# VainF/Diff-Pruning

Measured on NVIDIA H100. Metric: taylor_score_unet_fwd_bwd_passes_per_sec, higher is better.
Workload: dtype f32

## Files before the change

diff-pruning_b200/csrc/conv_tc.cu:

```cuda
#include <cuda.h>
#include <cuda_fp16.h>
#include <mutex>
#include "common.cuh"
#include "sm90.cuh"

namespace {
using namespace sm90;

constexpr int BM = 128, BK = 64;
constexpr int A_BYTES = BM * 32 * 4;

struct TcParams {
  int Nimg, H, W;
  int Nout;
  int kchunks;
  int bw, bh, bn, tiles_w, tiles_h;
  float* y; long long ldy;
  const float* bias;
  const float* rowadd; long long ld_rowadd;
  const float* residual; long long ld_res;
  int accumulate;
  int vec4;
  int ntaps;
  signed char dh[9], dw[9], wt[9];
  int os, oa, ob, Ho, Wo;
  int in_stride;
  float alpha;
  int b_from_img;
  const uint32_t* amax_a;
  const uint32_t* amax_b;
  uint32_t* amax_out;
  int ksplit, it_per_split;
  float* ws; long long ws_split_stride; int ws_ld;
};

__device__ __forceinline__ uint32_t smem_u32(const void* p) { return (uint32_t)__cvta_generic_to_shared(p); }
__device__ __forceinline__ void mbar_init(uint32_t bar, uint32_t count) {
  asm volatile("mbarrier.init.shared::cta.b64 [%0], %1;" ::"r"(bar), "r"(count));
}
__device__ __forceinline__ void mbar_expect_tx(uint32_t bar, uint32_t bytes) {
  asm volatile("mbarrier.arrive.expect_tx.shared::cta.b64 _, [%0], %1;" ::"r"(bar), "r"(bytes) : "memory");
}
__device__ __forceinline__ void mbar_arrive(uint32_t bar) {
  asm volatile("mbarrier.arrive.shared::cta.b64 _, [%0];" ::"r"(bar) : "memory");
}
__device__ __forceinline__ void mbar_wait(uint32_t bar, uint32_t parity) {
  uint32_t done;
  do {
    asm volatile(
        "{\n\t.reg .pred p;\n\t"
        "mbarrier.try_wait.parity.shared::cta.b64 p, [%1], %2;\n\t"
        "selp.u32 %0, 1, 0, p;\n\t}"
        : "=r"(done)
        : "r"(bar), "r"(parity)
        : "memory");
  } while (!done);
}
__device__ __forceinline__ void tma_load_4d(uint32_t dst, const CUtensorMap* map, uint32_t bar, int c0, int c1, int c2, int c3) {
  asm volatile(
      "cp.async.bulk.tensor.4d.shared::cluster.global.mbarrier::complete_tx::bytes [%0], [%1, {%3, %4, %5, %6}], [%2];"
      ::"r"(dst), "l"(reinterpret_cast<uint64_t>(map)), "r"(bar), "r"(c0), "r"(c1), "r"(c2), "r"(c3)
      : "memory");
}
__device__ __forceinline__ void tma_load_3d(uint32_t dst, const CUtensorMap* map, uint32_t bar, int c0, int c1, int c2) {
  asm volatile(
      "cp.async.bulk.tensor.3d.shared::cluster.global.mbarrier::complete_tx::bytes [%0], [%1, {%3, %4, %5}], [%2];"
      ::"r"(dst), "l"(reinterpret_cast<uint64_t>(map)), "r"(bar), "r"(c0), "r"(c1), "r"(c2)
      : "memory");
}
__device__ __forceinline__ int amax_exponent(const uint32_t* slot) {
  const int E = (int)((__ldg(slot) >> 23) & 0xFFu);
  return min(max(E, 14), 254);
}
__device__ __forceinline__ float scale_up(int E) { return __uint_as_float((uint32_t)(267 - E) << 23); }
__device__ __forceinline__ float scale_dn(int E) { return __uint_as_float((uint32_t)(E - 13) << 23); }
constexpr float LO_SCALE = 2048.f, LO_UNSCALE = 1.f / 2048.f;
__device__ __forceinline__ void split2(float a, float b, uint32_t& h, uint32_t& l) {
  const __half2 hh = __floats2half2_rn(a, b);
  const float2 hf = __half22float2(hh);
  const __half2 ll = __floats2half2_rn((a - hf.x) * LO_SCALE, (b - hf.y) * LO_SCALE);
  h = *reinterpret_cast<const uint32_t*>(&hh);
  l = *reinterpret_cast<const uint32_t*>(&ll);
}
__device__ __forceinline__ void split1(float v, __half& h, __half& l) {
  h = __float2half_rn(v);
  l = __float2half_rn((v - __half2float(h)) * LO_SCALE);
}

constexpr int PS_STAGES = 3, PS_BN = 128;
constexpr int PS_B_BYTES = PS_BN * BK * 2;
constexpr int PS_STAGE_BYTES = 2 * A_BYTES + 2 * PS_B_BYTES;

__global__ void __launch_bounds__(THREADS, 1)
conv_tc_ps_kernel(const __grid_constant__ CUtensorMap mapA, const __grid_constant__ CUtensorMap mapBh,
                  const __grid_constant__ CUtensorMap mapBl, const TcParams p, const int tiles_m, const int total_tiles) {
  const int total_work = total_tiles * p.ksplit;
  extern __shared__ uint8_t smem_raw[];
  const uint32_t raw = smem_u32(smem_raw);
  const uint32_t pad_to = ((raw + 1023u) & ~1023u) - raw;
  uint8_t* smem = smem_raw + pad_to;
  const uint32_t sbase = raw + pad_to;
  const uint32_t bar0 = sbase + PS_STAGES * PS_STAGE_BYTES;
  auto full_bar = [&](int s) { return bar0 + 8u * s; };
  auto empty_bar = [&](int s) { return bar0 + 8u * (PS_STAGES + s); };
  const int wg = threadIdx.x >> 7, tid = threadIdx.x & 127;
  if (threadIdx.x == 0) {
    for (int s = 0; s < PS_STAGES; ++s) { mbar_init(full_bar(s), 1); mbar_init(empty_bar(s), 8); }
    mbar_init_fence();
  }
  __syncthreads();
  const int iters_per_tile = p.ntaps * p.kchunks;

  auto tile_coords = [&](int tile, int& q0, int& p0, int& n0, int& nblk) {
    nblk = tile / tiles_m;
    const int tile_m = tile - nblk * tiles_m;
    const int tw = tile_m % p.tiles_w;
    const int th = (tile_m / p.tiles_w) % p.tiles_h;
    const int tn = tile_m / (p.tiles_w * p.tiles_h);
    q0 = tw * p.bw; p0 = th * p.bh; n0 = tn * p.bn;
  };

  if (wg == 0) {
    setmaxnreg_dec<40>();
    if (threadIdx.x == 0) {
      prefetch_map(&mapA); prefetch_map(&mapBh); prefetch_map(&mapBl);
      uint32_t g = 0;
      for (int wi = blockIdx.x; wi < total_work; wi += gridDim.x) {
        const int tile = wi % total_tiles, it0 = (wi / total_tiles) * p.it_per_split, it1 = min(iters_per_tile, it0 + p.it_per_split);
        int q0, p0, n0, nblk;
        tile_coords(tile, q0, p0, n0, nblk);
        for (int it = it0; it < it1; ++it, ++g) {
          const int s = g % PS_STAGES;
          const uint32_t ph = (g / PS_STAGES) & 1u;
          mbar_wait(empty_bar(s), ph ^ 1u);
          mbar_expect_tx(full_bar(s), PS_STAGE_BYTES);
          const int tap = it / p.kchunks, kc = it - tap * p.kchunks;
          const uint32_t st = sbase + s * PS_STAGE_BYTES;
          const int aw = q0 * p.in_stride + p.dw[tap], ah = p0 * p.in_stride + p.dh[tap];
          tma_load_4d(st, &mapA, full_bar(s), kc * BK, aw, ah, n0);
          tma_load_4d(st + A_BYTES, &mapA, full_bar(s), kc * BK + 32, aw, ah, n0);
          const int tapb = p.b_from_img ? n0 : p.wt[tap];
          tma_load_3d(st + 2 * A_BYTES, &mapBh, full_bar(s), kc * BK, nblk * PS_BN, tapb);
          tma_load_3d(st + 2 * A_BYTES + PS_B_BYTES, &mapBl, full_bar(s), kc * BK, nblk * PS_BN, tapb);
        }
      }
    }
    return;
  }
  setmaxnreg_inc<232>();
  const int c = wg - 1;
  const int warp = tid >> 5, lane = tid & 31;
  const int r = 64 * c + (tid & 63), h = tid >> 6;
  const uint32_t sw = (uint32_t)(r & 7);
  const float sa = scale_up(amax_exponent(p.amax_a));
  const float f1 = scale_dn(amax_exponent(p.amax_a)), f2 = scale_dn(amax_exponent(p.amax_b)) * p.alpha;
  auto fin = [&](float main, float corr) { return fmaf(corr, LO_UNSCALE, main) * f1 * f2; };
  float amax = 0.f;
  uint32_t g = 0;
  for (int wi = blockIdx.x; wi < total_work; wi += gridDim.x) {
    const int tile = wi % total_tiles, it0 = (wi / total_tiles) * p.it_per_split, it1 = min(iters_per_tile, it0 + p.it_per_split);
    float acc[64], cor[64];
    int prev_s = 0;
    for (int it = it0; it < it1; ++it, ++g) {
      const int s = g % PS_STAGES;
      const uint32_t ph = (g / PS_STAGES) & 1u;
      mbar_wait(full_bar(s), ph);
      uint8_t* a0 = smem + s * PS_STAGE_BYTES + r * 128;
      uint8_t* a1 = a0 + A_BYTES;
      const uint8_t* src = h ? a1 : a0;
      float4 v[8];
#pragma unroll
      for (int j = 0; j < 8; ++j) v[j] = *reinterpret_cast<const float4*>(src + ((j ^ sw) << 4));
      named_sync(1 + c, 128);
#pragma unroll
      for (int m = 0; m < 4; ++m) {
        const float4 x0 = v[2 * m], x1 = v[2 * m + 1];
        uint4 hq, lq;
        split2(x0.x * sa, x0.y * sa, hq.x, lq.x);
        split2(x0.z * sa, x0.w * sa, hq.y, lq.y);
        split2(x1.x * sa, x1.y * sa, hq.z, lq.z);
        split2(x1.z * sa, x1.w * sa, hq.w, lq.w);
        const uint32_t pos = (uint32_t)(((4 * h + m) ^ sw) << 4);
        *reinterpret_cast<uint4*>(a0 + pos) = hq;
        *reinterpret_cast<uint4*>(a1 + pos) = lq;
      }
      fence_proxy_async();
      named_sync(1 + c, 128);
      const uint32_t st = sbase + s * PS_STAGE_BYTES;
      wgmma_fence();
#pragma unroll
      for (int k = 0; k < BK / 16; ++k) {
        const uint64_t a_hi = desc_k(st + c * 8192 + k * 32), a_lo = desc_k(st + A_BYTES + c * 8192 + k * 32);
        const uint64_t b_hi = desc_k(st + 2 * A_BYTES + k * 32), b_lo = desc_k(st + 2 * A_BYTES + PS_B_BYTES + k * 32);
        const uint32_t first = (it > it0 || k > 0) ? 1u : 0u;
        wgmma_f16_n128<0, 0>(acc, a_hi, b_hi, first);
        wgmma_f16_n128<0, 0>(cor, a_hi, b_lo, first);
        wgmma_f16_n128<0, 0>(cor, a_lo, b_hi, 1u);
      }
      wgmma_commit();
      wgmma_wait<1>();
      if (it > it0 && lane == 0) mbar_arrive(empty_bar(prev_s));
      prev_s = s;
    }
    wgmma_wait<0>();
    fence_regs(acc); fence_regs(cor);
    if (lane == 0) mbar_arrive(empty_bar(prev_s));

    int q0, p0, n0, nblk;
    tile_coords(tile, q0, p0, n0, nblk);
#pragma unroll
    for (int i = 0; i < 2; ++i) {
      const int row = 64 * c + 16 * warp + (lane >> 2) + 8 * i;
      const int cb = 2 * (lane & 3);
      if (p.ksplit > 1) {
        float* wrow = p.ws + (long long)(wi / total_tiles) * p.ws_split_stride + ((long long)(tile - nblk * tiles_m) * BM + row) * p.ws_ld + nblk * PS_BN;
#pragma unroll
        for (int j = 0; j < 16; ++j)
          *reinterpret_cast<float2*>(wrow + 8 * j + cb) =
              make_float2(fin(acc[4 * j + 2 * i], cor[4 * j + 2 * i]), fin(acc[4 * j + 2 * i + 1], cor[4 * j + 2 * i + 1]));
        continue;
      }
      const int w_l = row % p.bw, h_l = (row / p.bw) % p.bh, n_l = row / (p.bw * p.bh);
      const int img = n0 + n_l;
      if (img >= p.Nimg) continue;
      const long long m = ((long long)img * p.Ho + ((p0 + h_l) * p.os + p.oa)) * p.Wo + ((q0 + w_l) * p.os + p.ob);
      float* yrow = p.y + m * p.ldy;
      const float* rrow = p.residual ? p.residual + m * p.ld_res : nullptr;
      const float* arow2 = p.rowadd ? p.rowadd + (long long)img * p.ld_rowadd : nullptr;
#pragma unroll
      for (int j = 0; j < 16; ++j) {
        const int col = nblk * PS_BN + 8 * j + cb;
        float o[2] = {fin(acc[4 * j + 2 * i], cor[4 * j + 2 * i]), fin(acc[4 * j + 2 * i + 1], cor[4 * j + 2 * i + 1])};
        if (p.vec4 && col + 2 <= p.Nout) {
          if (p.bias) { const float2 t = __ldg(reinterpret_cast<const float2*>(p.bias + col)); o[0] += t.x; o[1] += t.y; }
          if (arow2) { const float2 t = __ldg(reinterpret_cast<const float2*>(arow2 + col)); o[0] += t.x; o[1] += t.y; }
          if (rrow) { const float2 t = __ldg(reinterpret_cast<const float2*>(rrow + col)); o[0] += t.x; o[1] += t.y; }
          float2* dst = reinterpret_cast<float2*>(yrow + col);
          if (p.accumulate) { const float2 t = *dst; o[0] += t.x; o[1] += t.y; }
          *dst = make_float2(o[0], o[1]);
          amax = fmaxf(amax, fmaxf(fabsf(o[0]), fabsf(o[1])));
        } else {
#pragma unroll
          for (int e = 0; e < 2; ++e) {
            const int cc = col + e;
            if (cc < p.Nout) {
              float ov = o[e];
              if (p.bias) ov += __ldg(p.bias + cc);
              if (arow2) ov += __ldg(arow2 + cc);
              if (rrow) ov += __ldg(rrow + cc);
              if (p.accumulate) ov += yrow[cc];
              yrow[cc] = ov;
              amax = fmaxf(amax, fabsf(ov));
            }
          }
        }
      }
    }
  }
  if (p.amax_out && p.ksplit == 1) amax_commit(p.amax_out, amax);
}

__global__ void __launch_bounds__(256) splitk_epilogue_kernel(const TcParams p, const int tiles_m) {
  const int c4 = (p.Nout + 3) >> 2;
  const long long total = (long long)tiles_m * BM * c4;
  float amax = 0.f;
  for (long long i = blockIdx.x * 256ll + threadIdx.x; i < total; i += (long long)gridDim.x * 256) {
    const long long grow = i / c4;
    const int c = (int)(i - grow * c4) << 2;
    const int tile_m = (int)(grow / BM), row = (int)(grow - (long long)tile_m * BM);
    const int tw = tile_m % p.tiles_w, th = (tile_m / p.tiles_w) % p.tiles_h, tn = tile_m / (p.tiles_w * p.tiles_h);
    const int w_l = row % p.bw, h_l = (row / p.bw) % p.bh, n_l = row / (p.bw * p.bh);
    const int img = tn * p.bn + n_l;
    if (img >= p.Nimg) continue;
    const float* src = p.ws + grow * p.ws_ld + c;
    float4 acc = *reinterpret_cast<const float4*>(src);
    for (int ks = 1; ks < p.ksplit; ++ks) {
      const float4 t = *reinterpret_cast<const float4*>(src + ks * p.ws_split_stride);
      acc.x += t.x; acc.y += t.y; acc.z += t.z; acc.w += t.w;
    }
    float o[4] = {acc.x, acc.y, acc.z, acc.w};
    const long long m = ((long long)img * p.Ho + ((th * p.bh + h_l) * p.os + p.oa)) * p.Wo + ((tw * p.bw + w_l) * p.os + p.ob);
    float* yrow = p.y + m * p.ldy;
#pragma unroll
    for (int e = 0; e < 4; ++e) {
      const int cc = c + e;
      if (cc < p.Nout) {
        float v = o[e];
        if (p.bias) v += __ldg(p.bias + cc);
        if (p.rowadd) v += __ldg(p.rowadd + (long long)img * p.ld_rowadd + cc);
        if (p.residual) v += __ldg(p.residual + m * p.ld_res + cc);
        if (p.accumulate) v += yrow[cc];
        yrow[cc] = v;
        amax = fmaxf(amax, fabsf(v));
      }
    }
  }
  if (p.amax_out) amax_commit(p.amax_out, amax);
}

struct WgParams {
  int Nimg, H, W, C, K;
  int R, S, pad;
  int bw, bh, bn, tiles_w, tiles_h;
  int total_chunks, chunks_per_split;
  int c_tiles;
  float* ws;
  int in_stride;
  const uint32_t* amax_x; const uint32_t* amax_y;
  float* bias_ws;
};
constexpr int WG_KPIX = 64;
constexpr int WG_BLK = WG_KPIX * 128;
constexpr int WG_STAGES = 3, WG_STAGE_BYTES = 8 * WG_BLK;

__global__ void __launch_bounds__(THREADS, 1)
wgrad_tc_kernel(const __grid_constant__ CUtensorMap mapDy, const __grid_constant__ CUtensorMap mapX, const WgParams p) {
  extern __shared__ uint8_t smem_raw[];
  const uint32_t raw = smem_u32(smem_raw);
  const uint32_t pad_to = ((raw + 1023u) & ~1023u) - raw;
  uint8_t* smem = smem_raw + pad_to;
  const uint32_t sbase = raw + pad_to;
  const uint32_t bar0 = sbase + WG_STAGES * WG_STAGE_BYTES;
  auto full_bar = [&](int s) { return bar0 + 8u * s; };
  auto empty_bar = [&](int s) { return bar0 + 8u * (WG_STAGES + s); };
  float* bsh = reinterpret_cast<float*>(smem + WG_STAGES * WG_STAGE_BYTES + 8 * 2 * WG_STAGES);
  const int wg = threadIdx.x >> 7, tid = threadIdx.x & 127;
  if (threadIdx.x == 0) {
    for (int s = 0; s < WG_STAGES; ++s) { mbar_init(full_bar(s), 1); mbar_init(empty_bar(s), 8); }
    mbar_init_fence();
  }
  __syncthreads();

  const int T = p.R * p.S;
  int tile = blockIdx.x;
  const int tap = tile % T; tile /= T;
  const int ct = tile % p.c_tiles;
  const int kt = tile / p.c_tiles;
  const int r = tap / p.S, sx = tap - r * p.S;
  const int chunk0 = blockIdx.y * p.chunks_per_split;
  const int chunk1 = min(p.total_chunks, chunk0 + p.chunks_per_split);
  const int num_iters = max(0, chunk1 - chunk0);
  const int dy_boxes = min(4, (p.K - kt * 128 + 31) >> 5), x_boxes = min(4, (p.C - ct * 128 + 31) >> 5);

  if (wg == 0) {
    setmaxnreg_dec<40>();
    if (threadIdx.x == 0) {
      prefetch_map(&mapDy); prefetch_map(&mapX);
      for (int it = 0; it < num_iters; ++it) {
        const int s = it % WG_STAGES;
        const uint32_t ph = (uint32_t)(it / WG_STAGES) & 1u;
        mbar_wait(empty_bar(s), ph ^ 1u);
        mbar_expect_tx(full_bar(s), (uint32_t)((dy_boxes + x_boxes) * WG_BLK));
        const int chunk = chunk0 + it;
        const int tw = chunk % p.tiles_w;
        const int th = (chunk / p.tiles_w) % p.tiles_h;
        const int tn = chunk / (p.tiles_w * p.tiles_h);
        const int q0 = tw * p.bw, p0 = th * p.bh, n0 = tn * p.bn;
        const uint32_t st = sbase + s * WG_STAGE_BYTES;
        const int xw = q0 * p.in_stride + sx - p.pad, xh = p0 * p.in_stride + r - p.pad;
#pragma unroll
        for (int b = 0; b < 4; ++b) {
          const uint32_t slot = (uint32_t)((b & 1) * 2 + (b >> 1));
          if (b < dy_boxes) tma_load_4d(st + slot * WG_BLK, &mapDy, full_bar(s), kt * 128 + b * 32, q0, p0, n0);
          if (b < x_boxes) tma_load_4d(st + (4 + slot) * WG_BLK, &mapX, full_bar(s), ct * 128 + b * 32, xw, xh, n0);
        }
      }
    }
    return;
  }
  setmaxnreg_inc<232>();
  const int c = wg - 1;
  const int warp = tid >> 5, lane = tid & 31;
  const int Ey = amax_exponent(p.amax_y), Ex = amax_exponent(p.amax_x);
  const float sy = scale_up(Ey), sxs = scale_up(Ex);
  const int ch = tid & 63, dh = tid >> 6;
  const bool dy_valid = ((64 * c + ch) >> 5) < dy_boxes;
  const uint32_t dy_raw = (uint32_t)((ch >> 5) * 2 + c) * WG_BLK, bl = (uint32_t)(ch & 31);
  const int xp = tid & 63, xh = tid >> 6;
  const bool x_valid = 2 * c + xh < x_boxes;
  const uint32_t xsw = (uint32_t)(xp & 7);
  float bsum = 0.f;
  float acc[64], cor[64];
  int prev_s = 0;
  for (int it = 0; it < num_iters; ++it) {
    const int s = it % WG_STAGES;
    const uint32_t ph = (uint32_t)(it / WG_STAGES) & 1u;
    mbar_wait(full_bar(s), ph);
    uint8_t* stp = smem + s * WG_STAGE_BYTES;
    float dv[32];
    if (dy_valid) {
#pragma unroll
      for (int j = 0; j < 32; ++j) {
        const int pix = 32 * dh + j;
        dv[j] = *reinterpret_cast<const float*>(stp + dy_raw + pix * 128 + ((((bl >> 2) ^ (uint32_t)pix) & 7u) << 4) + (bl & 3u) * 4);
      }
    }
    uint8_t* x0 = stp + 4 * WG_BLK + c * WG_BLK + xp * 128;
    uint8_t* x1 = x0 + 2 * WG_BLK;
    float4 xv[8];
    if (x_valid) {
      const uint8_t* src = xh ? x1 : x0;
#pragma unroll
      for (int j = 0; j < 8; ++j) xv[j] = *reinterpret_cast<const float4*>(src + ((j ^ xsw) << 4));
    }
    named_sync(1 + c, 128);
    if (dy_valid) {
      __half* dh_hi = reinterpret_cast<__half*>(stp + c * WG_BLK);
      __half* dh_lo = reinterpret_cast<__half*>(stp + (2 + c) * WG_BLK);
      float ssum = 0.f;
#pragma unroll
      for (int j = 0; j < 32; j += 2) {
        ssum += dv[j] + dv[j + 1];
#pragma unroll
        for (int e = 0; e < 2; ++e) {
          const int pix = 32 * dh + j + e;
          const int off = pix * 64 + ((((ch >> 3) ^ pix) & 7) << 3) + (ch & 7);
          split1(dv[j + e] * sy, dh_hi[off], dh_lo[off]);
        }
      }
      bsum += ssum;
    }
    if (x_valid) {
#pragma unroll
      for (int m = 0; m < 4; ++m) {
        const float4 u0 = xv[2 * m], u1 = xv[2 * m + 1];
        uint4 hq, lq;
        split2(u0.x * sxs, u0.y * sxs, hq.x, lq.x);
        split2(u0.z * sxs, u0.w * sxs, hq.y, lq.y);
        split2(u1.x * sxs, u1.y * sxs, hq.z, lq.z);
        split2(u1.z * sxs, u1.w * sxs, hq.w, lq.w);
        const uint32_t pos = (uint32_t)(((4 * xh + m) ^ xsw) << 4);
        *reinterpret_cast<uint4*>(x0 + pos) = hq;
        *reinterpret_cast<uint4*>(x1 + pos) = lq;
      }
    }
    fence_proxy_async();
    named_sync(3, 256);
    const uint32_t st = sbase + s * WG_STAGE_BYTES;
    wgmma_fence();
#pragma unroll
    for (int k = 0; k < WG_KPIX / 16; ++k) {
      const uint64_t a_hi = desc_mn(st + c * WG_BLK + k * 2048, WG_BLK), a_lo = desc_mn(st + (2 + c) * WG_BLK + k * 2048, WG_BLK);
      const uint64_t b_hi = desc_mn(st + 4 * WG_BLK + k * 2048, WG_BLK), b_lo = desc_mn(st + 6 * WG_BLK + k * 2048, WG_BLK);
      const uint32_t first = (it > 0 || k > 0) ? 1u : 0u;
      wgmma_f16_n128<1, 1>(acc, a_hi, b_hi, first);
      wgmma_f16_n128<1, 1>(cor, a_hi, b_lo, first);
      wgmma_f16_n128<1, 1>(cor, a_lo, b_hi, 1u);
    }
    wgmma_commit();
    wgmma_wait<1>();
    if (it > 0 && lane == 0) mbar_arrive(empty_bar(prev_s));
    prev_s = s;
  }
  wgmma_wait<0>();
  fence_regs(acc); fence_regs(cor);
  if (dh) bsh[64 * c + ch] = bsum;
  named_sync(3, 256);
  if (!dh) {
    bsum += bsh[64 * c + ch];
    const int kout = kt * 128 + 64 * c + ch;
    if (p.bias_ws && tap == 0 && ct == 0 && kout < p.K) p.bias_ws[(long long)blockIdx.y * p.K + kout] = bsum;
  }
  const float f1 = scale_dn(Ey), f2 = scale_dn(Ex);
  const long long TC_ = (long long)T * p.C;
#pragma unroll
  for (int i = 0; i < 2; ++i) {
    const int kout = kt * 128 + 64 * c + 16 * warp + (lane >> 2) + 8 * i;
    if (kout >= p.K) continue;
    float* wrow = p.ws + ((long long)blockIdx.y * p.K + kout) * TC_ + (long long)tap * p.C;
#pragma unroll
    for (int j = 0; j < 16; ++j)
#pragma unroll
      for (int e = 0; e < 2; ++e) {
        const int col = ct * 128 + 8 * j + 2 * (lane & 3) + e;
        if (col < p.C) wrow[col] = num_iters ? fmaf(cor[4 * j + 2 * i + e], LO_UNSCALE, acc[4 * j + 2 * i + e]) * f1 * f2 : 0.f;
      }
  }
}

typedef CUresult (*EncodeTiledFn)(CUtensorMap*, CUtensorMapDataType, cuuint32_t, void*, const cuuint64_t*, const cuuint64_t*,
                                  const cuuint32_t*, const cuuint32_t*, CUtensorMapInterleave, CUtensorMapSwizzle,
                                  CUtensorMapL2promotion, CUtensorMapFloatOOBfill);
EncodeTiledFn g_encode = nullptr;
int g_tc_state = -1;
int g_num_sms = 132;
std::mutex g_tc_mutex;
constexpr int PS_SMEM = PS_STAGES * PS_STAGE_BYTES + 2048;
constexpr int WG_SMEM = WG_STAGES * WG_STAGE_BYTES + 2048;

static int wrow(int c) { return c > 64 ? ((c + 63) & ~63) : ((c + 7) & ~7); }

int tc_init() {
  std::lock_guard<std::mutex> lk(g_tc_mutex);
  if (g_tc_state >= 0) return g_tc_state;
  g_tc_state = 0;
  int dev = 0, major = 0;
  if (cudaGetDevice(&dev) != cudaSuccess) { (void)cudaGetLastError(); return 0; }
  if (cudaDeviceGetAttribute(&major, cudaDevAttrComputeCapabilityMajor, dev) != cudaSuccess || major != 9) { (void)cudaGetLastError(); return 0; }
  void* fn = nullptr;
  cudaDriverEntryPointQueryResult qres;
  if (cudaGetDriverEntryPoint("cuTensorMapEncodeTiled", &fn, cudaEnableDefault, &qres) != cudaSuccess || !fn ||
      qres != cudaDriverEntryPointSuccess) { (void)cudaGetLastError(); return 0; }
  g_encode = (EncodeTiledFn)fn;
  bool ok = cudaFuncSetAttribute(conv_tc_ps_kernel, cudaFuncAttributeMaxDynamicSharedMemorySize, PS_SMEM) == cudaSuccess;
  ok = ok && cudaFuncSetAttribute(wgrad_tc_kernel, cudaFuncAttributeMaxDynamicSharedMemorySize, WG_SMEM) == cudaSuccess;
  cudaDeviceGetAttribute(&g_num_sms, cudaDevAttrMultiProcessorCount, dev);
  if (!ok) { (void)cudaGetLastError(); return 0; }
  (void)cudaGetLastError();
  g_tc_state = 1;
  return 1;
}

bool make_map(CUtensorMap* m, const void* base, int rank, const cuuint64_t* dims, const cuuint64_t* strides_bytes,
              const cuuint32_t* box, CUtensorMapSwizzle swz = CU_TENSOR_MAP_SWIZZLE_128B, int pix_stride = 1,
              CUtensorMapDataType dtype = CU_TENSOR_MAP_DATA_TYPE_FLOAT32) {
  cuuint32_t estr[5] = {1, (cuuint32_t)pix_stride, (cuuint32_t)pix_stride, 1, 1};
  CUresult r = g_encode(m, dtype, (cuuint32_t)rank, const_cast<void*>(base), dims, strides_bytes, box, estr,
                        CU_TENSOR_MAP_INTERLEAVE_NONE, swz, CU_TENSOR_MAP_L2_PROMOTION_L2_256B,
                        CU_TENSOR_MAP_FLOAT_OOB_FILL_NONE);
  return r == CUDA_SUCCESS;
}

bool pick_box(int N, int H, int W, int& bw, int& bh, int& bn) {
  if (W >= BM) {
    if (W % BM) return false;
    bw = BM; bh = 1; bn = 1; return true;
  }
  if (BM % W) return false;
  bw = W;
  int rem = BM / W;
  if (H >= rem) {
    if (H % rem) return false;
    bh = rem; bn = 1; return true;
  }
  if (rem % H) return false;
  bh = H; bn = rem / H;
  return true;
}

struct TapTable { int n; signed char dh[9], dw[9], wt[9]; };
static int pick_ksplit(int tiles, int iters, int& it_per_split) {
  it_per_split = iters;
  if (tiles * 2 > g_num_sms || iters < 8) return 1;
  int ks = g_num_sms / tiles;
  if (ks > iters / 4) ks = iters / 4;
  if (ks > 16) ks = 16;
  if (ks < 2) return 1;
  it_per_split = (iters + ks - 1) / ks;
  return (iters + it_per_split - 1) / it_per_split;
}

int launch_tc(const float* act, long long ld_act, const uint32_t* amax_a, int Nimg, int H, int W, int Kg, const void* w_hi, const void* w_lo,
              const uint32_t* amax_b, int Nout, int T, const TapTable& taps, int os, int oa, int ob, int Ho, int Wo, float* out,
              long long ld_out, const float* bias, const float* rowadd, long long ld_rowadd, const float* residual, long long ld_res,
              int accumulate, cudaStream_t st, float alpha = 1.0f, int b_from_img = 0, int in_stride = 1, int ldb = -1, float* ws = nullptr,
              long long* ws_need = nullptr, uint32_t* amax_out = nullptr) {
  if (ldb < 0) ldb = wrow(Kg);
  if (!tc_init()) return DP_ERR_UNSUPPORTED;
  if (!ws_need && (!w_hi || !w_lo || !amax_a || !amax_b)) return DP_ERR_UNSUPPORTED;
  if (!ws_need && (ld_act % 4 || ((uintptr_t)act & 15) || ((uintptr_t)w_hi & 15) || ((uintptr_t)w_lo & 15))) return DP_ERR_UNSUPPORTED;
  int bw, bh, bn;
  if (!pick_box(Nimg, H, W, bw, bh, bn)) return DP_ERR_UNSUPPORTED;
  constexpr int BN = 128;
  if (ws_need) {
    *ws_need = 0;
    if (b_from_img) return DP_OK;
    const int tiles_m = (W / bw) * (H / bh) * ((Nimg + bn - 1) / bn), n_tiles = (Nout + 127) / 128;
    int ips;
    const int ks = pick_ksplit(tiles_m * n_tiles, taps.n * ((Kg + BK - 1) / BK), ips);
    if (ks > 1) *ws_need = (long long)ks * tiles_m * BM * n_tiles * 128;
    return DP_OK;
  }
  if (b_from_img && bn != 1) return DP_ERR_UNSUPPORTED;
  CUtensorMap mA, mBh, mBl;
  {
    const cuuint64_t Hin = (cuuint64_t)H * in_stride, Win = (cuuint64_t)W * in_stride;
    cuuint64_t dims[4] = {(cuuint64_t)Kg, Win, Hin, (cuuint64_t)Nimg};
    cuuint64_t str[3] = {(cuuint64_t)ld_act * 4, Win * ld_act * 4, Hin * Win * ld_act * 4};
    cuuint32_t box[4] = {32u, (cuuint32_t)(bw * in_stride), (cuuint32_t)(bh * in_stride), (cuuint32_t)bn};
    if (box[1] > 256 || box[2] > 256) return DP_ERR_UNSUPPORTED;
    if (!make_map(&mA, act, 4, dims, str, box, CU_TENSOR_MAP_SWIZZLE_128B, in_stride)) return DP_ERR_UNSUPPORTED;
  }
  {
    const cuuint64_t Kp = (cuuint64_t)ldb;
    if (Kp % 8) return DP_ERR_UNSUPPORTED;
    cuuint64_t dims[3] = {Kp, (cuuint64_t)Nout, (cuuint64_t)T};
    cuuint64_t str[2] = {Kp * 2, (cuuint64_t)Nout * Kp * 2};
    cuuint32_t box[3] = {(cuuint32_t)BK, (cuuint32_t)BN, 1};
    if (!make_map(&mBh, w_hi, 3, dims, str, box, CU_TENSOR_MAP_SWIZZLE_128B, 1, CU_TENSOR_MAP_DATA_TYPE_FLOAT16) ||
        !make_map(&mBl, w_lo, 3, dims, str, box, CU_TENSOR_MAP_SWIZZLE_128B, 1, CU_TENSOR_MAP_DATA_TYPE_FLOAT16)) return DP_ERR_UNSUPPORTED;
  }
  TcParams p{};
  p.Nimg = Nimg; p.H = H; p.W = W; p.Nout = Nout;
  p.ntaps = taps.n;
  for (int i = 0; i < 9; ++i) { p.dh[i] = taps.dh[i]; p.dw[i] = taps.dw[i]; p.wt[i] = taps.wt[i]; }
  p.os = os; p.oa = oa; p.ob = ob; p.Ho = Ho; p.Wo = Wo;
  p.alpha = alpha; p.b_from_img = b_from_img; p.in_stride = in_stride; p.amax_a = amax_a; p.amax_b = amax_b; p.amax_out = amax_out;
  p.kchunks = (Kg + BK - 1) / BK;
  p.bw = bw; p.bh = bh; p.bn = bn; p.tiles_w = W / bw; p.tiles_h = H / bh;
  p.y = out; p.ldy = ld_out; p.bias = bias; p.rowadd = rowadd; p.ld_rowadd = ld_rowadd; p.residual = residual; p.ld_res = ld_res;
  p.accumulate = accumulate;
  auto al16 = [](const void* q, long long ld) { return q == nullptr || ((((uintptr_t)q) & 15) == 0 && (ld % 4) == 0); };
  p.vec4 = (al16(out, ld_out) && al16(bias, 0) && al16(rowadd, ld_rowadd) && al16(residual, ld_res)) ? 1 : 0;
  const int tiles_n = (Nimg + bn - 1) / bn;
  dim3 grid((unsigned)(p.tiles_w * p.tiles_h * tiles_n), (unsigned)((Nout + BN - 1) / BN));
  p.ksplit = 1; p.it_per_split = p.ntaps * p.kchunks;
  {
    const int tiles_m = (int)grid.x, total = (int)(grid.x * grid.y);
    if (ws && !b_from_img) {
      p.ksplit = pick_ksplit(total, p.ntaps * p.kchunks, p.it_per_split);
      p.ws = ws; p.ws_ld = (int)grid.y * 128; p.ws_split_stride = (long long)tiles_m * BM * p.ws_ld;
    }
    const int work = total * p.ksplit;
    const int ctas = work < g_num_sms ? work : g_num_sms;
    conv_tc_ps_kernel<<<ctas, THREADS, PS_SMEM, st>>>(mA, mBh, mBl, p, tiles_m, total);
    if (p.ksplit > 1) {
      int rc = dp_check_launch();
      if (rc) return rc;
      const long long items = (long long)tiles_m * BM * ((Nout + 3) / 4);
      long long blocks = (items + 255) / 256;
      if (blocks > g_num_sms * 8) blocks = g_num_sms * 8;
      splitk_epilogue_kernel<<<(int)blocks, 256, 0, st>>>(p, tiles_m);
    }
  }
  return dp_check_launch();
}

__global__ void pack_tc_kernel(const float* __restrict__ w, int K, int C, int RS, int Cp, int Kp, __half* __restrict__ kc_hi,
                               __half* __restrict__ kc_lo, __half* __restrict__ ck_hi, __half* __restrict__ ck_lo,
                               const uint32_t* __restrict__ amax) {
  const float sw = scale_up(amax_exponent(amax));
  const long long na = (long long)RS * K * Cp, nb = (long long)RS * C * Kp;
  const long long total = na > nb ? na : nb;
  for (long long i = blockIdx.x * (long long)blockDim.x + threadIdx.x; i < total; i += (long long)gridDim.x * blockDim.x) {
    if (i < na && kc_hi) {
      int c = (int)(i % Cp); long long t = i / Cp; int k = (int)(t % K), tap = (int)(t / K);
      split1(c < C ? w[((long long)k * C + c) * RS + tap] * sw : 0.f, kc_hi[i], kc_lo[i]);
    }
    if (i < nb && ck_hi) {
      int k = (int)(i % Kp); long long t = i / Kp; int c = (int)(t % C), tap = (int)(t / C);
      split1(k < K ? w[((long long)k * C + c) * RS + tap] * sw : 0.f, ck_hi[i], ck_lo[i]);
    }
  }
}
__global__ void split_h3_rows_kernel(const float* __restrict__ x, long long ld, long long bs, int rows, int cols, int pitch, int vec,
                                     __half* __restrict__ hi, __half* __restrict__ lo, const uint32_t* __restrict__ amax) {
  const float sx = scale_up(amax_exponent(amax));
  const int groups = pitch >> 3;
  const long long total = (long long)rows * groups;
  const float* xb = x + (long long)blockIdx.y * bs;
  __half* hb = hi + (long long)blockIdx.y * rows * pitch;
  __half* lb = lo + (long long)blockIdx.y * rows * pitch;
  for (long long i = blockIdx.x * 256ll + threadIdx.x; i < total; i += (long long)gridDim.x * 256) {
    const long long r = i / groups;
    const int c0 = (int)(i - r * groups) << 3;
    const float* src = xb + r * ld + c0;
    float v[8];
    if (vec && c0 + 8 <= cols) {
      const float4 a = __ldg(reinterpret_cast<const float4*>(src)), b = __ldg(reinterpret_cast<const float4*>(src + 4));
      v[0] = a.x; v[1] = a.y; v[2] = a.z; v[3] = a.w; v[4] = b.x; v[5] = b.y; v[6] = b.z; v[7] = b.w;
    } else {
#pragma unroll
      for (int j = 0; j < 8; ++j) v[j] = (c0 + j < cols) ? __ldg(src + j) : 0.f;
    }
    uint4 h, l;
    split2(v[0] * sx, v[1] * sx, h.x, l.x); split2(v[2] * sx, v[3] * sx, h.y, l.y);
    split2(v[4] * sx, v[5] * sx, h.z, l.z); split2(v[6] * sx, v[7] * sx, h.w, l.w);
    *reinterpret_cast<uint4*>(hb + r * pitch + c0) = h;
    *reinterpret_cast<uint4*>(lb + r * pitch + c0) = l;
  }
}
__global__ void __launch_bounds__(256) split_h3_t_kernel(const float* __restrict__ x, long long ld, long long bs, int rows, int cols, int vec,
                                                         __half* __restrict__ hi, __half* __restrict__ lo, const uint32_t* __restrict__ amax) {
  __shared__ float t[64][65];
  const float sx = scale_up(amax_exponent(amax));
  const int b = blockIdx.z, r0 = blockIdx.y * 64, c0 = blockIdx.x * 64, tid = threadIdx.x;
  const float* xb = x + (long long)b * bs;
  {
    const int cc = (tid & 15) * 4, c = c0 + cc;
#pragma unroll
    for (int i = 0; i < 4; ++i) {
      const int rr = (tid >> 4) + 16 * i, r = r0 + rr;
      float4 v = make_float4(0.f, 0.f, 0.f, 0.f);
      if (r < rows) {
        const float* src = xb + (long long)r * ld + c;
        if (vec && c + 4 <= cols) v = __ldg(reinterpret_cast<const float4*>(src));
        else {
          if (c < cols) v.x = __ldg(src);
          if (c + 1 < cols) v.y = __ldg(src + 1);
          if (c + 2 < cols) v.z = __ldg(src + 2);
          if (c + 3 < cols) v.w = __ldg(src + 3);
        }
      }
      t[rr][cc] = v.x * sx; t[rr][cc + 1] = v.y * sx; t[rr][cc + 2] = v.z * sx; t[rr][cc + 3] = v.w * sx;
    }
  }
  __syncthreads();
  const int rows8 = (rows + 7) & ~7;
  const int c = c0 + (tid >> 2), rs = (tid & 3) * 16;
  if (c < cols) {
    const long long o = ((long long)b * cols + c) * rows8 + r0 + rs;
#pragma unroll
    for (int h8 = 0; h8 < 2; ++h8) {
      if (r0 + rs + 8 * h8 + 8 <= rows8) {
        uint4 h, l;
        const int rb = rs + 8 * h8, cl = tid >> 2;
        split2(t[rb][cl], t[rb + 1][cl], h.x, l.x); split2(t[rb + 2][cl], t[rb + 3][cl], h.y, l.y);
        split2(t[rb + 4][cl], t[rb + 5][cl], h.z, l.z); split2(t[rb + 6][cl], t[rb + 7][cl], h.w, l.w);
        *reinterpret_cast<uint4*>(hi + o + 8 * h8) = h;
        *reinterpret_cast<uint4*>(lo + o + 8 * h8) = l;
      }
    }
  }
}
__global__ void __launch_bounds__(256) transpose_batched_kernel(const float* __restrict__ in, float* __restrict__ out, int rows, int cols, int vec) {
  __shared__ float t[64][65];
  const int b = blockIdx.z, r0 = blockIdx.y * 64, c0 = blockIdx.x * 64, tid = threadIdx.x;
  const float* ib = in + (long long)b * rows * cols;
  float* ob = out + (long long)b * rows * cols;
  const int q4 = (tid & 15) * 4, l16 = tid >> 4;
#pragma unroll
  for (int i = 0; i < 4; ++i) {
    const int rr = l16 + 16 * i, r = r0 + rr, c = c0 + q4;
    float4 v = make_float4(0.f, 0.f, 0.f, 0.f);
    if (r < rows) {
      const float* src = ib + (long long)r * cols + c;
      if (vec && c + 4 <= cols) v = __ldg(reinterpret_cast<const float4*>(src));
      else {
        if (c < cols) v.x = __ldg(src);
        if (c + 1 < cols) v.y = __ldg(src + 1);
        if (c + 2 < cols) v.z = __ldg(src + 2);
        if (c + 3 < cols) v.w = __ldg(src + 3);
      }
    }
    t[rr][q4] = v.x; t[rr][q4 + 1] = v.y; t[rr][q4 + 2] = v.z; t[rr][q4 + 3] = v.w;
  }
  __syncthreads();
#pragma unroll
  for (int i = 0; i < 4; ++i) {
    const int cc = l16 + 16 * i, c = c0 + cc, r = r0 + q4;
    if (c < cols) {
      float* dst = ob + (long long)c * rows + r;
      if (vec && r + 4 <= rows) *reinterpret_cast<float4*>(dst) = make_float4(t[q4][cc], t[q4 + 1][cc], t[q4 + 2][cc], t[q4 + 3][cc]);
      else {
        if (r < rows) dst[0] = t[q4][cc];
        if (r + 1 < rows) dst[1] = t[q4 + 1][cc];
        if (r + 2 < rows) dst[2] = t[q4 + 2][cc];
        if (r + 3 < rows) dst[3] = t[q4 + 3][cc];
      }
    }
  }
}
}

extern "C" int dp_split_h3(const float* x, int64_t ld, int64_t bs, int32_t batch, int32_t rows, int32_t cols, int32_t transpose,
                           const uint32_t* amax, void* hi, void* lo, dp_stream_t stream) {
  DP_REQUIRE(x && hi && lo && amax, DP_ERR_NULL);
  DP_REQUIRE(batch > 0 && rows > 0 && cols > 0 && ld >= cols && batch <= 65535, DP_ERR_SHAPE);
  if (!transpose) {
    const int pitch = (cols + 7) & ~7;
    const int vec = ((((uintptr_t)x) & 15) == 0 && ld % 4 == 0 && bs % 4 == 0) ? 1 : 0;
    long long blocks = ((long long)rows * (pitch >> 3) + 255) / 256;
    if (blocks > g_num_sms * 8) blocks = g_num_sms * 8;
    split_h3_rows_kernel<<<dim3((unsigned)blocks, (unsigned)batch), 256, 0, (cudaStream_t)stream>>>(x, ld, bs, rows, cols, pitch, vec, (__half*)hi,
                                                                                                (__half*)lo, amax);
  } else {
    const int vec = ((((uintptr_t)x) & 15) == 0 && ld % 4 == 0 && bs % 4 == 0) ? 1 : 0;
    DP_REQUIRE((((uintptr_t)hi) & 15) == 0 && (((uintptr_t)lo) & 15) == 0, DP_ERR_ALIGN);
    dim3 grid((cols + 63) / 64, (((rows + 7) & ~7) + 63) / 64, batch);
    split_h3_t_kernel<<<grid, 256, 0, (cudaStream_t)stream>>>(x, ld, bs, rows, cols, vec, (__half*)hi, (__half*)lo, amax);
  }
// ... 176 lines not shown
```

diff-pruning_b200/csrc/sm90.cuh:

```cuda
#pragma once
#include <cuda.h>
#include <stdint.h>

namespace sm90 {

constexpr int THREADS = 384;

__device__ __forceinline__ void mbar_init_fence() { asm volatile("fence.mbarrier_init.release.cluster;" ::: "memory"); }
__device__ __forceinline__ void prefetch_map(const CUtensorMap* map) {
  asm volatile("prefetch.tensormap [%0];" ::"l"(reinterpret_cast<uint64_t>(map)) : "memory");
}
__device__ __forceinline__ void named_sync(int id, int count) { asm volatile("bar.sync %0, %1;" ::"r"(id), "r"(count) : "memory"); }
__device__ __forceinline__ void fence_proxy_async() { asm volatile("fence.proxy.async.shared::cta;" ::: "memory"); }

template <int N>
__device__ __forceinline__ void setmaxnreg_inc() { asm volatile("setmaxnreg.inc.sync.aligned.u32 %0;" ::"n"(N)); }
template <int N>
__device__ __forceinline__ void setmaxnreg_dec() { asm volatile("setmaxnreg.dec.sync.aligned.u32 %0;" ::"n"(N)); }

__device__ __forceinline__ uint64_t desc_k(uint32_t saddr) {
  return (uint64_t)((saddr & 0x3FFFF) >> 4) | (1ull << 16) | (64ull << 32) | (1ull << 62);
}
__device__ __forceinline__ uint64_t desc_mn(uint32_t saddr, uint32_t lbo_bytes) {
  return (uint64_t)((saddr & 0x3FFFF) >> 4) | ((uint64_t)(lbo_bytes >> 4) << 16) | (64ull << 32) | (1ull << 62);
}

__device__ __forceinline__ void wgmma_fence() { asm volatile("wgmma.fence.sync.aligned;" ::: "memory"); }
__device__ __forceinline__ void wgmma_commit() { asm volatile("wgmma.commit_group.sync.aligned;" ::: "memory"); }
template <int N>
__device__ __forceinline__ void wgmma_wait() { asm volatile("wgmma.wait_group.sync.aligned %0;" ::"n"(N) : "memory"); }
template <int R>
__device__ __forceinline__ void fence_regs(float (&d)[R]) {
#pragma unroll
  for (int i = 0; i < R; ++i) asm volatile("" : "+f"(d[i])::"memory");
}

#define DP_F4(i) "+f"(d[i]), "+f"(d[i + 1]), "+f"(d[i + 2]), "+f"(d[i + 3])
#define DP_F32(i) DP_F4(i), DP_F4(i + 4), DP_F4(i + 8), DP_F4(i + 12), DP_F4(i + 16), DP_F4(i + 20), DP_F4(i + 24), DP_F4(i + 28)
template <int TA, int TB>
__device__ __forceinline__ void wgmma_f16_n128(float (&d)[64], uint64_t a, uint64_t b, uint32_t acc) {
  asm volatile(
      "{\n\t.reg .pred p;\n\tsetp.ne.b32 p, %66, 0;\n\t"
      "wgmma.mma_async.sync.aligned.m64n128k16.f32.f16.f16 "
      "{%0, %1, %2, %3, %4, %5, %6, %7, %8, %9, %10, %11, %12, %13, %14, %15, "
      "%16, %17, %18, %19, %20, %21, %22, %23, %24, %25, %26, %27, %28, %29, %30, %31, "
      "%32, %33, %34, %35, %36, %37, %38, %39, %40, %41, %42, %43, %44, %45, %46, %47, "
      "%48, %49, %50, %51, %52, %53, %54, %55, %56, %57, %58, %59, %60, %61, %62, %63}, "
      "%64, %65, p, 1, 1, %67, %68;\n\t}"
      : DP_F32(0), DP_F32(32)
      : "l"(a), "l"(b), "r"(acc), "n"(TA), "n"(TB));
}
template <int TA, int TB>
__device__ __forceinline__ void wgmma_bf16_n64(float (&d)[32], uint64_t a, uint64_t b, uint32_t acc) {
  asm volatile(
      "{\n\t.reg .pred p;\n\tsetp.ne.b32 p, %34, 0;\n\t"
      "wgmma.mma_async.sync.aligned.m64n64k16.f32.bf16.bf16 "
      "{%0, %1, %2, %3, %4, %5, %6, %7, %8, %9, %10, %11, %12, %13, %14, %15, "
      "%16, %17, %18, %19, %20, %21, %22, %23, %24, %25, %26, %27, %28, %29, %30, %31}, "
      "%32, %33, p, 1, 1, %35, %36;\n\t}"
      : DP_F32(0)
      : "l"(a), "l"(b), "r"(acc), "n"(TA), "n"(TB));
}
template <int TA, int TB>
__device__ __forceinline__ void wgmma_bf16_n128(float (&d)[64], uint64_t a, uint64_t b, uint32_t acc) {
  asm volatile(
      "{\n\t.reg .pred p;\n\tsetp.ne.b32 p, %66, 0;\n\t"
      "wgmma.mma_async.sync.aligned.m64n128k16.f32.bf16.bf16 "
      "{%0, %1, %2, %3, %4, %5, %6, %7, %8, %9, %10, %11, %12, %13, %14, %15, "
      "%16, %17, %18, %19, %20, %21, %22, %23, %24, %25, %26, %27, %28, %29, %30, %31, "
      "%32, %33, %34, %35, %36, %37, %38, %39, %40, %41, %42, %43, %44, %45, %46, %47, "
      "%48, %49, %50, %51, %52, %53, %54, %55, %56, %57, %58, %59, %60, %61, %62, %63}, "
      "%64, %65, p, 1, 1, %67, %68;\n\t}"
      : DP_F32(0), DP_F32(32)
      : "l"(a), "l"(b), "r"(acc), "n"(TA), "n"(TB));
}
template <int TA, int TB>
__device__ __forceinline__ void wgmma_bf16_n192(float (&d)[96], uint64_t a, uint64_t b, uint32_t acc) {
  asm volatile(
      "{\n\t.reg .pred p;\n\tsetp.ne.b32 p, %98, 0;\n\t"
      "wgmma.mma_async.sync.aligned.m64n192k16.f32.bf16.bf16 "
      "{%0, %1, %2, %3, %4, %5, %6, %7, %8, %9, %10, %11, %12, %13, %14, %15, "
      "%16, %17, %18, %19, %20, %21, %22, %23, %24, %25, %26, %27, %28, %29, %30, %31, "
      "%32, %33, %34, %35, %36, %37, %38, %39, %40, %41, %42, %43, %44, %45, %46, %47, "
      "%48, %49, %50, %51, %52, %53, %54, %55, %56, %57, %58, %59, %60, %61, %62, %63, "
      "%64, %65, %66, %67, %68, %69, %70, %71, %72, %73, %74, %75, %76, %77, %78, %79, "
      "%80, %81, %82, %83, %84, %85, %86, %87, %88, %89, %90, %91, %92, %93, %94, %95}, "
      "%96, %97, p, 1, 1, %99, %100;\n\t}"
      : DP_F32(0), DP_F32(32), DP_F32(64)
      : "l"(a), "l"(b), "r"(acc), "n"(TA), "n"(TB));
}
template <int TA, int TB>
__device__ __forceinline__ void wgmma_bf16_n256(float (&d)[128], uint64_t a, uint64_t b, uint32_t acc) {
  asm volatile(
      "{\n\t.reg .pred p;\n\tsetp.ne.b32 p, %130, 0;\n\t"
      "wgmma.mma_async.sync.aligned.m64n256k16.f32.bf16.bf16 "
      "{%0, %1, %2, %3, %4, %5, %6, %7, %8, %9, %10, %11, %12, %13, %14, %15, "
      "%16, %17, %18, %19, %20, %21, %22, %23, %24, %25, %26, %27, %28, %29, %30, %31, "
      "%32, %33, %34, %35, %36, %37, %38, %39, %40, %41, %42, %43, %44, %45, %46, %47, "
      "%48, %49, %50, %51, %52, %53, %54, %55, %56, %57, %58, %59, %60, %61, %62, %63, "
      "%64, %65, %66, %67, %68, %69, %70, %71, %72, %73, %74, %75, %76, %77, %78, %79, "
      "%80, %81, %82, %83, %84, %85, %86, %87, %88, %89, %90, %91, %92, %93, %94, %95, "
      "%96, %97, %98, %99, %100, %101, %102, %103, %104, %105, %106, %107, %108, %109, %110, %111, "
      "%112, %113, %114, %115, %116, %117, %118, %119, %120, %121, %122, %123, %124, %125, %126, %127}, "
      "%128, %129, p, 1, 1, %131, %132;\n\t}"
      : DP_F32(0), DP_F32(32), DP_F32(64), DP_F32(96)
      : "l"(a), "l"(b), "r"(acc), "n"(TA), "n"(TB));
}
template <int N, int TA, int TB>
__device__ __forceinline__ void wgmma_bf16(float (&d)[N / 2], uint64_t a, uint64_t b, uint32_t acc) {
  if constexpr (N == 64) wgmma_bf16_n64<TA, TB>(d, a, b, acc);
  else if constexpr (N == 128) wgmma_bf16_n128<TA, TB>(d, a, b, acc);
  else if constexpr (N == 192) wgmma_bf16_n192<TA, TB>(d, a, b, acc);
  else wgmma_bf16_n256<TA, TB>(d, a, b, acc);
}

}
```

Before: 21.45.

## Feed wgrad dy operand from registers via RS wgmma instead of shared memory

The weight-gradient kernel now loads dy values straight into register fragments in the wgmma A-operand layout, splits them into fp16 hi/lo in registers, and issues register-sourced wgmma instead of writing split halves back to shared memory. The bias sum is reduced with warp shuffles instead of a shared-memory exchange. Fragments are double-buffered across two unrolled stages. Producer and consumer register limits are rebalanced to fit the extra fragment registers. This removes the smem write/read round trip for the A operand, at the cost of higher register pressure and the risk of spilling.

```diff
diff --git a/diff-pruning_b200/csrc/conv_tc.cu b/diff-pruning_b200/csrc/conv_tc.cu
--- a/diff-pruning_b200/csrc/conv_tc.cu
+++ b/diff-pruning_b200/csrc/conv_tc.cu
@@ -323,7 +323,6 @@
   const uint32_t bar0 = sbase + WG_STAGES * WG_STAGE_BYTES;
   auto full_bar = [&](int s) { return bar0 + 8u * s; };
   auto empty_bar = [&](int s) { return bar0 + 8u * (WG_STAGES + s); };
-  float* bsh = reinterpret_cast<float*>(smem + WG_STAGES * WG_STAGE_BYTES + 8 * 2 * WG_STAGES);
   const int wg = threadIdx.x >> 7, tid = threadIdx.x & 127;
   if (threadIdx.x == 0) {
     for (int s = 0; s < WG_STAGES; ++s) { mbar_init(full_bar(s), 1); mbar_init(empty_bar(s), 8); }
@@ -343,7 +342,7 @@
   const int dy_boxes = min(4, (p.K - kt * 128 + 31) >> 5), x_boxes = min(4, (p.C - ct * 128 + 31) >> 5);
 
   if (wg == 0) {
-    setmaxnreg_dec<40>();
+    setmaxnreg_dec<24>();
     if (threadIdx.x == 0) {
       prefetch_map(&mapDy); prefetch_map(&mapX);
       for (int it = 0; it < num_iters; ++it) {
@@ -368,33 +367,25 @@
     }
     return;
   }
-  setmaxnreg_inc<232>();
+  setmaxnreg_inc<240>();
   const int c = wg - 1;
   const int warp = tid >> 5, lane = tid & 31;
   const int Ey = amax_exponent(p.amax_y), Ex = amax_exponent(p.amax_x);
   const float sy = scale_up(Ey), sxs = scale_up(Ex);
-  const int ch = tid & 63, dh = tid >> 6;
-  const bool dy_valid = ((64 * c + ch) >> 5) < dy_boxes;
-  const uint32_t dy_raw = (uint32_t)((ch >> 5) * 2 + c) * WG_BLK, bl = (uint32_t)(ch & 31);
+  const bool dy_valid = 2 * c + (warp >> 1) < dy_boxes;
+  const uint32_t cb = (uint32_t)(16 * (warp & 1) + (lane >> 2)), pe = (uint32_t)(2 * (lane & 3));
+  const uint32_t dy_off = (uint32_t)((warp >> 1) * 2 + c) * WG_BLK + pe * 128 + (((cb >> 2) ^ pe) << 4) + (cb & 3) * 4;
   const int xp = tid & 63, xh = tid >> 6;
   const bool x_valid = 2 * c + xh < x_boxes;
   const uint32_t xsw = (uint32_t)(xp & 7);
-  float bsum = 0.f;
+  float bsum[2] = {0.f, 0.f};
   float acc[64], cor[64];
   int prev_s = 0;
-  for (int it = 0; it < num_iters; ++it) {
+  auto stage = [&](uint32_t (&fah)[4][4], uint32_t (&fal)[4][4], const int it) {
     const int s = it % WG_STAGES;
     const uint32_t ph = (uint32_t)(it / WG_STAGES) & 1u;
     mbar_wait(full_bar(s), ph);
     uint8_t* stp = smem + s * WG_STAGE_BYTES;
-    float dv[32];
-    if (dy_valid) {
-#pragma unroll
-      for (int j = 0; j < 32; ++j) {
-        const int pix = 32 * dh + j;
-        dv[j] = *reinterpret_cast<const float*>(stp + dy_raw + pix * 128 + ((((bl >> 2) ^ (uint32_t)pix) & 7u) << 4) + (bl & 3u) * 4);
-      }
-    }
     uint8_t* x0 = stp + 4 * WG_BLK + c * WG_BLK + xp * 128;
     uint8_t* x1 = x0 + 2 * WG_BLK;
     float4 xv[8];
@@ -404,22 +395,6 @@
       for (int j = 0; j < 8; ++j) xv[j] = *reinterpret_cast<const float4*>(src + ((j ^ xsw) << 4));
     }
     named_sync(1 + c, 128);
-    if (dy_valid) {
-      __half* dh_hi = reinterpret_cast<__half*>(stp + c * WG_BLK);
-      __half* dh_lo = reinterpret_cast<__half*>(stp + (2 + c) * WG_BLK);
-      float ssum = 0.f;
-#pragma unroll
-      for (int j = 0; j < 32; j += 2) {
-        ssum += dv[j] + dv[j + 1];
-#pragma unroll
-        for (int e = 0; e < 2; ++e) {
-          const int pix = 32 * dh + j + e;
-          const int off = pix * 64 + ((((ch >> 3) ^ pix) & 7) << 3) + (ch & 7);
-          split1(dv[j + e] * sy, dh_hi[off], dh_lo[off]);
-        }
-      }
-      bsum += ssum;
-    }
     if (x_valid) {
 #pragma unroll
       for (int m = 0; m < 4; ++m) {
@@ -436,30 +411,51 @@
     }
     fence_proxy_async();
     named_sync(3, 256);
+    if (dy_valid) {
+#pragma unroll
+      for (int k = 0; k < WG_KPIX / 16; ++k)
+#pragma unroll
+        for (int q = 0; q < 4; ++q) {
+          const uint8_t* d = stp + (16 * k + 8 * (q >> 1)) * 128;
+          const float v0 = *reinterpret_cast<const float*>(d + (dy_off ^ (32u * (q & 1))));
+          const float v1 = *reinterpret_cast<const float*>(d + (dy_off ^ (32u * (q & 1) + 144u)));
+          bsum[q & 1] += v0 + v1;
+          split2(v0 * sy, v1 * sy, fah[k][q], fal[k][q]);
+        }
+    } else {
+#pragma unroll
+      for (int k = 0; k < WG_KPIX / 16; ++k)
+#pragma unroll
+        for (int q = 0; q < 4; ++q) fah[k][q] = fal[k][q] = 0u;
+    }
     const uint32_t st = sbase + s * WG_STAGE_BYTES;
     wgmma_fence();
 #pragma unroll
     for (int k = 0; k < WG_KPIX / 16; ++k) {
-      const uint64_t a_hi = desc_mn(st + c * WG_BLK + k * 2048, WG_BLK), a_lo = desc_mn(st + (2 + c) * WG_BLK + k * 2048, WG_BLK);
       const uint64_t b_hi = desc_mn(st + 4 * WG_BLK + k * 2048, WG_BLK), b_lo = desc_mn(st + 6 * WG_BLK + k * 2048, WG_BLK);
       const uint32_t first = (it > 0 || k > 0) ? 1u : 0u;
-      wgmma_f16_n128<1, 1>(acc, a_hi, b_hi, first);
-      wgmma_f16_n128<1, 1>(cor, a_hi, b_lo, first);
-      wgmma_f16_n128<1, 1>(cor, a_lo, b_hi, 1u);
+      wgmma_f16_n128_rs<1>(acc, fah[k], b_hi, first);
+      wgmma_f16_n128_rs<1>(cor, fah[k], b_lo, first);
+      wgmma_f16_n128_rs<1>(cor, fal[k], b_hi, 1u);
     }
     wgmma_commit();
     wgmma_wait<1>();
     if (it > 0 && lane == 0) mbar_arrive(empty_bar(prev_s));
     prev_s = s;
-  }
+  };
+  uint32_t fah0[4][4], fal0[4][4], fah1[4][4], fal1[4][4];
+  int it = 0;
+  for (; it + 1 < num_iters; it += 2) {
+    stage(fah0, fal0, it);
+    stage(fah1, fal1, it + 1);
+  }
+  if (it < num_iters) stage(fah0, fal0, it);
   wgmma_wait<0>();
   fence_regs(acc); fence_regs(cor);
-  if (dh) bsh[64 * c + ch] = bsum;
-  named_sync(3, 256);
-  if (!dh) {
-    bsum += bsh[64 * c + ch];
-    const int kout = kt * 128 + 64 * c + ch;
-    if (p.bias_ws && tap == 0 && ct == 0 && kout < p.K) p.bias_ws[(long long)blockIdx.y * p.K + kout] = bsum;
+#pragma unroll
+  for (int i = 0; i < 2; ++i) {
+    bsum[i] += __shfl_xor_sync(0xffffffffu, bsum[i], 1);
+    bsum[i] += __shfl_xor_sync(0xffffffffu, bsum[i], 2);
   }
   const float f1 = scale_dn(Ey), f2 = scale_dn(Ex);
   const long long TC_ = (long long)T * p.C;
@@ -467,6 +463,7 @@
   for (int i = 0; i < 2; ++i) {
     const int kout = kt * 128 + 64 * c + 16 * warp + (lane >> 2) + 8 * i;
     if (kout >= p.K) continue;
+    if (p.bias_ws && tap == 0 && ct == 0 && (lane & 3) == 0) p.bias_ws[(long long)blockIdx.y * p.K + kout] = bsum[i];
     float* wrow = p.ws + ((long long)blockIdx.y * p.K + kout) * TC_ + (long long)tap * p.C;
 #pragma unroll
     for (int j = 0; j < 16; ++j)
diff --git a/diff-pruning_b200/csrc/sm90.cuh b/diff-pruning_b200/csrc/sm90.cuh
--- a/diff-pruning_b200/csrc/sm90.cuh
+++ b/diff-pruning_b200/csrc/sm90.cuh
@@ -49,6 +49,19 @@
       "%64, %65, p, 1, 1, %67, %68;\n\t}"
       : DP_F32(0), DP_F32(32)
       : "l"(a), "l"(b), "r"(acc), "n"(TA), "n"(TB));
+}
+template <int TB>
+__device__ __forceinline__ void wgmma_f16_n128_rs(float (&d)[64], const uint32_t (&a)[4], uint64_t b, uint32_t acc) {
+  asm volatile(
+      "{\n\t.reg .pred p;\n\tsetp.ne.b32 p, %69, 0;\n\t"
+      "wgmma.mma_async.sync.aligned.m64n128k16.f32.f16.f16 "
+      "{%0, %1, %2, %3, %4, %5, %6, %7, %8, %9, %10, %11, %12, %13, %14, %15, "
+      "%16, %17, %18, %19, %20, %21, %22, %23, %24, %25, %26, %27, %28, %29, %30, %31, "
+      "%32, %33, %34, %35, %36, %37, %38, %39, %40, %41, %42, %43, %44, %45, %46, %47, "
+      "%48, %49, %50, %51, %52, %53, %54, %55, %56, %57, %58, %59, %60, %61, %62, %63}, "
+      "{%64, %65, %66, %67}, %68, p, 1, 1, %70;\n\t}"
+      : DP_F32(0), DP_F32(32)
+      : "r"(a[0]), "r"(a[1]), "r"(a[2]), "r"(a[3]), "l"(b), "r"(acc), "n"(TB));
 }
 template <int TA, int TB>
 __device__ __forceinline__ void wgmma_bf16_n64(float (&d)[32], uint64_t a, uint64_t b, uint32_t acc) {
```

Result: faster. 22.32, median of 6 (+4.0%).
